# TechnetiumMan/DiffSound

Hardware: AMD Instinct MI355X
Metric: fwd+bwd modal-analysis passes/sec, 100k-tet ord-2 mesh, 64 modes (higher is better)
Workload: dtype f32

## Files before the change

diffsound_amd/csrc/spmm_narrow.inc:

```
constexpr int NARROW_TILE = 320;

template <bool SCALAR, int LVL>
__global__ void __launch_bounds__(256)
    spmm_union_narrow_kernel(const int2* __restrict__ utab, const int4* __restrict__ ctab, unsigned ngroups,
                             const int32_t* __restrict__ gent, const float* __restrict__ vals, int64_t nv,
                             const float* __restrict__ X, int64_t ldx, float* __restrict__ Y, int64_t ldy, int ncols, unsigned nwg) {
    using f4 = __attribute__((ext_vector_type(4))) float;
    __shared__ int s_ent[4][NARROW_TILE];
    __shared__ int s_pre[4][NARROW_TILE];
    const int lane = threadIdx.x & 63;
    const int wave = __builtin_amdgcn_readfirstlane(threadIdx.x >> 6);
    const unsigned grp = ds::xcd_remap(blockIdx.x, nwg) * 4 + wave;
    if (grp >= ngroups) return;
    int ch0 = (int)grp, ch1 = (int)grp + 1;
    if (utab) {
        const int2 ut = utab[grp];
        ch0 = __builtin_amdgcn_readfirstlane(ut.x), ch1 = __builtin_amdgcn_readfirstlane(ut.y);
    }
    const int4 cf = ctab[ch0];
    const int e0 = __builtin_amdgcn_readfirstlane(cf.x);
    const int b0 = __builtin_amdgcn_readfirstlane(cf.z);
    const int e1 = ch1 - 1 == ch0 ? __builtin_amdgcn_readfirstlane(cf.y) : __builtin_amdgcn_readfirstlane(ctab[ch1 - 1].y);
    const int ne = e1 - e0;
    const int cq = ncols >> 2;
    const int sh = cq == 1 ? 0 : (cq == 2 ? 1 : 2);
    const int cl = lane & ((1 << sh) - 1), es = lane >> sh, nslot = 64 >> sh;
    const bool active = cl < cq;
    int* se = s_ent[wave];
    int* sp = s_pre[wave];
    f4 acc[4][3];
#pragma unroll
    for (int s = 0; s < 4; ++s)
#pragma unroll
        for (int i = 0; i < 3; ++i) acc[s][i] = f4{0.f, 0.f, 0.f, 0.f};
    int base_blk = b0;
    for (int t0 = 0; t0 < ne; t0 += NARROW_TILE) {
        const int nt = min(NARROW_TILE, ne - t0);
        int running = 0;
        for (int i = 0; i < nt; i += 64) {
            const int idx = i + lane;
            const int ent = idx < nt ? gent[e0 + t0 + idx] : 0;
            const int pc = __builtin_popcount((unsigned)ent >> 28);
            int incl = pc;
#pragma unroll
            for (int d = 1; d < 64; d <<= 1) {
                const int v = __shfl_up(incl, d);
                if (lane >= d) incl += v;
            }
            if (idx < nt) se[idx] = ent, sp[idx] = running + incl - pc;
            running += __shfl(incl, 63);
        }
        __builtin_amdgcn_fence(__ATOMIC_RELEASE, "wavefront");
        __builtin_amdgcn_wave_barrier();
        __builtin_amdgcn_fence(__ATOMIC_ACQUIRE, "wavefront");
        for (int e = es; e < nt; e += nslot) {
            const int ent = se[e];
            const unsigned m = (unsigned)ent >> 28;
            const int64_t col = ent & 0x0fffffff;
            int64_t blk = base_blk + sp[e];
            f4 x0 = {0.f, 0.f, 0.f, 0.f}, x1 = x0, x2 = x0;
            if (active) {
                const float* xp = X + col * 3 * ldx + cl * 4;
                x0 = *reinterpret_cast<const f4*>(xp);
                x1 = *reinterpret_cast<const f4*>(xp + ldx);
                x2 = *reinterpret_cast<const f4*>(xp + 2 * ldx);
            }
#pragma unroll
            for (int s = 0; s < 4; ++s) {
                if (m & (1u << s)) {
                    if constexpr (SCALAR) {
                        const float c = vals[blk];
                        acc[s][0] += c * x0, acc[s][1] += c * x1, acc[s][2] += c * x2;
                    } else {
                        const float* k = vals + blk * 9;
                        float kk[9];
#pragma unroll
                        for (int j = 0; j < 9; ++j) kk[j] = k[j];
#pragma unroll
                        for (int i = 0; i < 3; ++i) acc[s][i] += kk[i] * x0 + kk[3 + i] * x1 + kk[6 + i] * x2;
                    }
                    ++blk;
                }
            }
        }
        base_blk += running;
        __builtin_amdgcn_fence(__ATOMIC_RELEASE, "wavefront");
        __builtin_amdgcn_wave_barrier();
        __builtin_amdgcn_fence(__ATOMIC_ACQUIRE, "wavefront");
    }
#pragma unroll
    for (int d = 1; d < 64; d <<= 1) {
        if (d >= (1 << sh)) {
#pragma unroll
            for (int s = 0; s < 4; ++s)
#pragma unroll
                for (int i = 0; i < 3; ++i)
#pragma unroll
                    for (int c = 0; c < 4; ++c) acc[s][i][c] += __shfl_xor(acc[s][i][c], d);
        }
    }
    const int64_t n0 = (int64_t)grp * 4;
    const int nn = (int)min<int64_t>(4, nv - n0);
    if (es == 0 && active) {
#pragma unroll
        for (int s = 0; s < 4; ++s)
            if (s < nn) {
#pragma unroll
                for (int i = 0; i < 3; ++i) *reinterpret_cast<f4*>(Y + ((n0 + s) * 3 + i) * ldy + cl * 4) = acc[s][i];
            }
    }
}
```

diffsound_amd/csrc/spmm_union.hip:

```cpp
#include <algorithm>
#include <cstdint>
#include <type_traits>

#include "spmm_device.h"

namespace {
#include "spmm_union.inc"
#include "spmm_narrow.inc"
}

__global__ void pack_groups_kernel(const float* __restrict__ vals_t, const int32_t* __restrict__ kperm, int64_t nnzb,
                                   float* __restrict__ kgrp) {
    const int64_t i = (int64_t)blockIdx.x * blockDim.x + threadIdx.x;
    if (i >= nnzb * 9) return;
    const int64_t p = i / 9;
    kgrp[i] = vals_t[(int64_t)kperm[p] * 9 + (i - p * 9)];
}

extern "C" int ds_pack_groups(const float* vals_t, const int32_t* kperm, int64_t nnzb, float* kgrp,
                              ds_stream_t stream) {
    DS_REQUIRE(vals_t && kperm && kgrp && nnzb > 0, "ds_pack_groups: bad argument");
    pack_groups_kernel<<<(unsigned)ds::ceil_div(nnzb * 9, 256), 256, 0, ds::as_stream(stream)>>>(vals_t, kperm, nnzb,
                                                                                                kgrp);
    DS_LAUNCH_CHECK("pack_groups_kernel");
    return DS_OK;
}

static int check_union_shape(const char* who, int64_t ngroups, int cap_blocks, int64_t nnzb, int64_t nv, int ncols,
                             const char* cap_note = "") {
    DS_REQUIRE(nv > 0 && ngroups == (nv + 3) / 4 && nnzb > 0 && ncols > 0 && ncols % 4 == 0 && ncols <= 84,
               "%s: ncols must be a multiple of 4 <= 84 and ngroups = ceil(nv / 4)", who);
    DS_REQUIRE(cap_blocks > 0 && cap_blocks <= UN_CAPB, "%s: a chunk of %d blocks exceeds the LDS image%s", who, cap_blocks, cap_note);
    return DS_OK;
}

extern "C" int ds_spmm_union(int epilogue, int level_tag, const int32_t* utab, const int32_t* ctab, int64_t ngroups, int cap_blocks,
                             const int32_t* gent,
                             const float* kgrp, int64_t nnzb, int64_t nv, const float* X, int64_t ldx, float* Y,
                             int64_t ldy, const float* R0, int64_t ldr, const float* dinv, int ncols, float c1, float c2,
                             int first, const float* Wprev, int64_t ldp, ds_stream_t stream) {
    DS_REQUIRE(ctab && gent && kgrp && X && Y, "ds_spmm_union: null pointer");
    DS_REQUIRE(epilogue >= 0 && epilogue <= 3, "ds_spmm_union: bad epilogue %d", epilogue);
    DS_REQUIRE(level_tag == 0 || level_tag == 1, "ds_spmm_union: level_tag must be 0 (fine) or 1 (corner-node level)");
    DS_REQUIRE(epilogue == 0 || epilogue == 3 || R0, "ds_spmm_union: the epilogue needs R0");
    DS_REQUIRE(epilogue != 1 || dinv, "ds_spmm_union: the Chebyshev epilogue needs dinv");
    if (int rc = check_union_shape("ds_spmm_union", ngroups, cap_blocks, nnzb, nv, ncols, " (DS_UNION_CAP = 140)")) return rc;
    DS_REQUIRE(ldx >= ncols && ldy >= ncols && (epilogue == 0 || epilogue == 3 || ldr >= ncols),
               "ds_spmm_union: leading dimension smaller than ncols");
    DS_REQUIRE(X != Y, "ds_spmm_union: X and Y must be different buffers");
    DS_REQUIRE(ldx * 12 < (int64_t)PIPE_OOB && ldy * 12 < (int64_t)PIPE_OOB && ldr * 12 < (int64_t)PIPE_OOB &&
                   nv * 36 < (int64_t)PIPE_OOB,
               "ds_spmm_union: a 3-row panel of %lld bytes exceeds the descriptor range", (long long)(ldx * 12));
    DS_REQUIRE(nnzb * 36 < ((int64_t)1 << 32), "ds_spmm_union: value array exceeds the descriptor range");
    uintptr_t al = reinterpret_cast<uintptr_t>(X) | reinterpret_cast<uintptr_t>(Y) | (uintptr_t)(ldx * 4) |
                   (uintptr_t)(ldy * 4) | reinterpret_cast<uintptr_t>(kgrp) | reinterpret_cast<uintptr_t>(ctab);
    if (epilogue == 1 || epilogue == 2) al |= reinterpret_cast<uintptr_t>(R0) | (uintptr_t)(ldr * 4);
    DS_REQUIRE((al & 15) == 0, "ds_spmm_union: rows, kgrp and ctab must be 16-byte aligned");
    hipStream_t st = ds::as_stream(stream);
    ChebEpilogue epi{R0, ldr, dinv, c1, c2, first};
    if (Wprev && epilogue == 1) {
        DS_REQUIRE(ldp >= ncols && ldp * 12 < (int64_t)PIPE_OOB &&
                       ((reinterpret_cast<uintptr_t>(Wprev) | (uintptr_t)(ldp * 4)) & 15) == 0 && Wprev != X,
                   "ds_spmm_union: bad W_prev block");
        epi.wprev = Wprev, epi.ldp = ldp;
    }
    const int lpn = ncols / 4;
    const int pkind = epilogue == 1 ? DS_PROF_TERM : (epilogue == 0 ? DS_PROF_KX : (epilogue == 3 ? DS_PROF_MX : -1));
    ds::ProfScope prof(pkind < 0 ? nullptr : stream, pkind < 0 ? 0 : pkind, nv, nnzb, ncols, (first ? 1 : 0) | (4 << 8));
#define DS_U(L, E) return launch_union<L, E>(utab, ctab, ngroups, cap_blocks, gent, kgrp, nnzb, nv, X, ldx, Y, ldy, lpn, st, epi)
#define DS_UL(L, E) do { if (level_tag == 1) return launch_union<L, E, false, true, 1>(utab, ctab, ngroups, cap_blocks, gent, kgrp, nnzb, nv, X, ldx, Y, ldy, lpn, st, epi); \
                         return launch_union<L, E, false, true, 0>(utab, ctab, ngroups, cap_blocks, gent, kgrp, nnzb, nv, X, ldx, Y, ldy, lpn, st, epi); } while (0)
    if (lpn == 20) {
        if (epilogue == 1) DS_U(20, 1);
        if (epilogue == 2) DS_U(20, 2);
        if (epilogue == 3) DS_UL(20, 3);
        DS_UL(20, 0);
    }
    if (epilogue == 1) DS_U(0, 1);
    if (epilogue == 2) DS_U(0, 2);
    if (epilogue == 3) DS_UL(0, 3);
    DS_UL(0, 0);
#undef DS_UL
#undef DS_U
}

extern "C" int ds_spmm_union_narrow(int kind, int level_tag, const int32_t* utab, const int32_t* ctab, int64_t ngroups,
                                    const int32_t* gent, const float* vals, int64_t nnzb, int64_t nv, const float* X, int64_t ldx,
                                    float* Y, int64_t ldy, int ncols, ds_stream_t stream) {
    DS_REQUIRE(ctab && gent && vals && X && Y, "ds_spmm_union_narrow: null pointer");
    DS_REQUIRE(kind == 0 || kind == 3, "ds_spmm_union_narrow: kind must be 0 (3x3 blocks) or 3 (node-scalar values)");
    DS_REQUIRE(level_tag == 0 || level_tag == 1, "ds_spmm_union_narrow: level_tag must be 0 (fine) or 1 (corner-node level)");
    DS_REQUIRE(nv > 0 && ngroups == (nv + 3) / 4 && nnzb > 0 && ncols > 0 && ncols % 4 == 0 && ncols <= 16,
               "ds_spmm_union_narrow: ncols must be a multiple of 4 <= 16 and ngroups = ceil(nv / 4)");
    DS_REQUIRE(ldx >= ncols && ldy >= ncols, "ds_spmm_union_narrow: leading dimension smaller than ncols");
    DS_REQUIRE(X != Y, "ds_spmm_union_narrow: X and Y must be different buffers");
    const uintptr_t al = reinterpret_cast<uintptr_t>(X) | reinterpret_cast<uintptr_t>(Y) | (uintptr_t)(ldx * 4) | (uintptr_t)(ldy * 4) |
                         reinterpret_cast<uintptr_t>(ctab);
    DS_REQUIRE((al & 15) == 0, "ds_spmm_union_narrow: rows and ctab must be 16-byte aligned");
    hipStream_t st = ds::as_stream(stream);
    const unsigned nwg = (unsigned)ds::ceil_div(ngroups, 4);
    ds::ProfScope prof(stream, kind == 0 ? DS_PROF_KX : DS_PROF_MX, nv, nnzb, ncols, 4 << 8);
#define DS_UN(S, V) spmm_union_narrow_kernel<S, V><<<nwg, 256, 0, st>>>(reinterpret_cast<const int2*>(utab), reinterpret_cast<const int4*>(ctab), \
                                                                       (unsigned)ngroups, gent, vals, nv, X, ldx, Y, ldy, ncols, nwg)
    if (kind == 0) {
        if (level_tag == 1) DS_UN(false, 1);
        else DS_UN(false, 0);
    } else {
        if (level_tag == 1) DS_UN(true, 1);
        else DS_UN(true, 0);
    }
#undef DS_UN
    DS_LAUNCH_CHECK("spmm_union_narrow_kernel");
    return DS_OK;
}

extern "C" int64_t ds_union_residual_workspace_bytes(int64_t ngroups, int ncols) {
    return ngroups * 2 * (int64_t)ncols * 4 + (int64_t)UN_NORM_BLOCKS * 2 * ncols * 8;
}

static int union_residual(const char* who, int level_tag, const int32_t* utab, const int32_t* ctab, int64_t ngroups, int cap_blocks,
                          const int32_t* gent, const float* kgrp, const float* mgrp, int64_t nnzb, int64_t nv, const float* X,
                          int64_t ldx, const double* lam, float* R, int64_t ldr, const float* dinv, float c, void* R16,
                          int64_t ldr16, void* W1, int64_t ldw1, int ncols, void* work, int64_t work_bytes, double* rn2,
                          double* xn2, ds_stream_t stream) {
    const bool pre = R16 != nullptr;
    DS_REQUIRE(ctab && gent && kgrp && mgrp && X && lam && (pre ? (W1 && dinv) : R != nullptr) && work && rn2 && xn2, "%s: null pointer", who);
    DS_REQUIRE(level_tag == 0 || (level_tag == 1 && !pre), "%s: level_tag must be 0 (fine)%s", who, pre ? "" : " or 1 (corner-node level)");
    if (int rc = check_union_shape(who, ngroups, cap_blocks, nnzb, nv, ncols)) return rc;
    uintptr_t al = reinterpret_cast<uintptr_t>(X) | (uintptr_t)(ldx * 4) | reinterpret_cast<uintptr_t>(kgrp) |
                   reinterpret_cast<uintptr_t>(ctab) | reinterpret_cast<uintptr_t>(work);
    if (pre) {
        DS_REQUIRE(ldx >= ncols && ldr16 >= ncols && ldw1 >= ncols, "%s: leading dimension smaller than ncols", who);
        DS_REQUIRE(R16 != W1 && R16 != X && W1 != X, "%s: X, R16 and W1 must be different buffers", who);
        DS_REQUIRE(ldx * 12 < (int64_t)PIPE_OOB && nv * 36 < (int64_t)PIPE_OOB && nnzb * 36 < ((int64_t)1 << 32),
                   "%s: operand beyond the descriptor range", who);
        const uintptr_t al8 = reinterpret_cast<uintptr_t>(R16) | reinterpret_cast<uintptr_t>(W1) | (uintptr_t)(ldr16 * 2) | (uintptr_t)(ldw1 * 2);
        DS_REQUIRE((al8 & 7) == 0 && (reinterpret_cast<uintptr_t>(dinv) & 3) == 0, "%s: bf16 rows must be 8-byte aligned", who);
    } else {
        DS_REQUIRE(ldx >= ncols && ldr >= ncols, "%s: leading dimension smaller than ncols", who);
        DS_REQUIRE(X != R, "%s: X and R must be different buffers", who);
        DS_REQUIRE(ldx * 12 < (int64_t)PIPE_OOB && ldr * 12 < (int64_t)PIPE_OOB && nnzb * 36 < ((int64_t)1 << 32),
                   "%s: operand beyond the descriptor range", who);
        al |= reinterpret_cast<uintptr_t>(R) | (uintptr_t)(ldr * 4);
    }
    DS_REQUIRE((al & 15) == 0, "%s: rows, kgrp, ctab and the workspace must be 16-byte aligned", who);
    DS_REQUIRE(work_bytes >= ds_union_residual_workspace_bytes(ngroups, ncols), "%s: workspace of %lld bytes needed", who,
               (long long)ds_union_residual_workspace_bytes(ngroups, ncols));
    hipStream_t st = ds::as_stream(stream);
    ChebEpilogue epi{nullptr, 0, pre ? dinv : nullptr, 0.f, pre ? c : 0.f, 0};
    epi.mvals = mgrp, epi.lam = lam, epi.nwork = static_cast<float*>(work);
    epi.w1 = W1, epi.ldw1 = ldw1;
    float* Y = pre ? static_cast<float*>(R16) : R;
    const int64_t ldy = pre ? ldr16 : ldr;
    const int lpn = ncols / 4;
    int rc;
    {
    ds::ProfScope prof(stream, DS_PROF_RESID, nv, nnzb, ncols, 4 << 8);
#define DS_UR(L, E, V) rc = launch_union<L, E, false, true, V>(utab, ctab, ngroups, cap_blocks, gent, kgrp, nnzb, nv, X, ldx, Y, ldy, lpn, st, epi)
    if (lpn == 20) {
        if (pre) DS_UR(20, 6, 0);
        else if (level_tag == 1) DS_UR(20, 4, 1);
        else DS_UR(20, 4, 0);
    } else {
        if (pre) DS_UR(0, 6, 0);
        else if (level_tag == 1) DS_UR(0, 4, 1);
        else DS_UR(0, 4, 0);
    }
#undef DS_UR
    }
    if (rc != DS_OK) return rc;
    double* partial = reinterpret_cast<double*>(static_cast<char*>(work) + ngroups * 2 * (int64_t)ncols * 4);
    union_norm_partial_kernel<<<UN_NORM_BLOCKS, 256, 0, st>>>(static_cast<const float*>(work), (unsigned)ngroups, 2 * ncols, partial);
    DS_LAUNCH_CHECK("union_norm_partial_kernel");
    union_norm_final_kernel<<<(unsigned)(2 * ncols), 256, 0, st>>>(partial, ncols, rn2, xn2);
    DS_LAUNCH_CHECK("union_norm_final_kernel");
    return DS_OK;
}

extern "C" int ds_union_residual(int level_tag, const int32_t* utab, const int32_t* ctab, int64_t ngroups, int cap_blocks,
                                 const int32_t* gent, const float* kgrp, const float* mgrp, int64_t nnzb, int64_t nv,
                                 const float* X, int64_t ldx, const double* lam, float* R, int64_t ldr, int ncols, void* work,
                                 int64_t work_bytes, double* rn2, double* xn2, ds_stream_t stream) {
    return union_residual("ds_union_residual", level_tag, utab, ctab, ngroups, cap_blocks, gent, kgrp, mgrp, nnzb, nv, X, ldx, lam, R,
                          ldr, nullptr, 0.f, nullptr, 0, nullptr, 0, ncols, work, work_bytes, rn2, xn2, stream);
}

extern "C" int ds_union_residual_pre(int level_tag, const int32_t* utab, const int32_t* ctab, int64_t ngroups, int cap_blocks,
                                     const int32_t* gent, const float* kgrp, const float* mgrp, int64_t nnzb, int64_t nv,
                                     const float* X, int64_t ldx, const double* lam, const float* dinv, float c, void* R16,
                                     int64_t ldr16, void* W1, int64_t ldw1, int ncols, void* work, int64_t work_bytes,
                                     double* rn2, double* xn2, ds_stream_t stream) {
    DS_REQUIRE(R16, "ds_union_residual_pre: null pointer");
    return union_residual("ds_union_residual_pre", level_tag, utab, ctab, ngroups, cap_blocks, gent, kgrp, mgrp, nnzb, nv, X, ldx, lam,
                          nullptr, 0, dinv, c, R16, ldr16, W1, ldw1, ncols, work, work_bytes, rn2, xn2, stream);
}

extern "C" int ds_spmm_union_km(int level_tag, const int32_t* utab, const int32_t* ctab, int64_t ngroups, int cap_blocks,
                                const int32_t* gent, const float* kgrp, const float* mgrp, int64_t nnzb, int64_t nv,
                                const float* X, int64_t ldx, float* KX, int64_t ldk, float* MX, int64_t ldm, int ncols,
                                ds_stream_t stream) {
    DS_REQUIRE(ctab && gent && kgrp && mgrp && X && KX && MX, "ds_spmm_union_km: null pointer");
    DS_REQUIRE(level_tag == 0 || level_tag == 1, "ds_spmm_union_km: level_tag must be 0 (fine) or 1 (corner-node level)");
    if (int rc = check_union_shape("ds_spmm_union_km", ngroups, cap_blocks, nnzb, nv, ncols)) return rc;
    DS_REQUIRE(ldx >= ncols && ldk >= ncols && ldm >= ncols, "ds_spmm_union_km: leading dimension smaller than ncols");
    DS_REQUIRE(X != KX && X != MX && KX != MX, "ds_spmm_union_km: X, KX and MX must be different buffers");
    DS_REQUIRE(ldx * 12 < (int64_t)PIPE_OOB && nnzb * 36 < ((int64_t)1 << 32), "ds_spmm_union_km: operand beyond the descriptor range");
    const uintptr_t al = reinterpret_cast<uintptr_t>(X) | reinterpret_cast<uintptr_t>(KX) | reinterpret_cast<uintptr_t>(MX) |
                         (uintptr_t)(ldx * 4) | (uintptr_t)(ldk * 4) | (uintptr_t)(ldm * 4) | reinterpret_cast<uintptr_t>(kgrp) |
                         reinterpret_cast<uintptr_t>(ctab);
    DS_REQUIRE((al & 15) == 0, "ds_spmm_union_km: rows, kgrp and ctab must be 16-byte aligned");
    hipStream_t st = ds::as_stream(stream);
    ChebEpilogue epi{nullptr, ldm, nullptr, 0.f, 0.f, 0};
    epi.mvals = mgrp, epi.nwork = MX;
    const int lpn = ncols / 4;
    ds::ProfScope prof(stream, DS_PROF_KM, nv, nnzb, ncols, 4 << 8);
#define DS_UKM(L, V) return launch_union<L, 5, false, true, V>(utab, ctab, ngroups, cap_blocks, gent, kgrp, nnzb, nv, X, ldx, KX, ldk, lpn, st, epi)
    if (lpn == 20) {
        if (level_tag == 1) DS_UKM(20, 1);
        DS_UKM(20, 0);
    }
    if (level_tag == 1) DS_UKM(0, 1);
    DS_UKM(0, 0);
#undef DS_UKM
}

extern "C" int ds_spmm_union16(int epilogue, const int32_t* utab, const int32_t* ctab, int64_t ngroups, int cap_blocks,
                               const int32_t* gent, const float* kgrp, int64_t nnzb, int64_t nv, const void* X,
                               int64_t ldx, void* Y, int64_t ldy, int y_f32, const void* R0, int64_t ldr,
                               const float* dinv, int ncols, float c1, float c2, int first, const void* Wprev,
                               int64_t ldp, ds_stream_t stream) {
    DS_REQUIRE(ctab && gent && kgrp && X && Y && R0, "ds_spmm_union16: null pointer");
    DS_REQUIRE(epilogue == 1 || epilogue == 2, "ds_spmm_union16: epilogue must be 1 (Chebyshev term) or 2 (residual)");
    DS_REQUIRE(epilogue != 1 || dinv, "ds_spmm_union16: the Chebyshev epilogue needs dinv");
    if (int rc = check_union_shape("ds_spmm_union16", ngroups, cap_blocks, nnzb, nv, ncols)) return rc;
    DS_REQUIRE(ldx >= ncols && ldy >= ncols && ldr >= ncols, "ds_spmm_union16: leading dimension smaller than ncols");
    DS_REQUIRE(X != Y, "ds_spmm_union16: X and Y must be different buffers");
    DS_REQUIRE(3 * nv * std::max(std::max(ldx, ldr), ldp) * 2 < (int64_t)PIPE_OOB && nv * 36 < (int64_t)PIPE_OOB,
               "ds_spmm_union16: a bf16 operand block of %lld bytes exceeds the descriptor range",
               (long long)(3 * nv * std::max(std::max(ldx, ldr), ldp) * 2));
    DS_REQUIRE(nnzb * 36 < ((int64_t)1 << 32), "ds_spmm_union16: value array exceeds the descriptor range");
    uintptr_t al = reinterpret_cast<uintptr_t>(X) | reinterpret_cast<uintptr_t>(R0) | (uintptr_t)(ldx * 2) | (uintptr_t)(ldr * 2);
    al |= reinterpret_cast<uintptr_t>(Y) | (uintptr_t)(ldy * (y_f32 ? 4 : 2));
    DS_REQUIRE((al & 7) == 0 && (!y_f32 || ((reinterpret_cast<uintptr_t>(Y) | (uintptr_t)(ldy * 4)) & 15) == 0) &&
                   ((reinterpret_cast<uintptr_t>(kgrp) | reinterpret_cast<uintptr_t>(ctab)) & 15) == 0,
               "ds_spmm_union16: bf16 rows must be 8-byte aligned (fp32 output rows, kgrp and ctab 16-byte)");
    hipStream_t st = ds::as_stream(stream);
    ChebEpilogue epi{static_cast<const float*>(R0), ldr, dinv, c1, c2, first};
    if (Wprev && epilogue == 1) {
        DS_REQUIRE(ldp >= ncols && ((reinterpret_cast<uintptr_t>(Wprev) | (uintptr_t)(ldp * 2)) & 7) == 0 && Wprev != X,
                   "ds_spmm_union16: bad W_prev block");
        epi.wprev = static_cast<const float*>(Wprev), epi.ldp = ldp;
    }
    DS_REQUIRE(!y_f32 || epilogue == 1, "ds_spmm_union16: an fp32 result is the Chebyshev term's only");
    const float* Xf = static_cast<const float*>(X);
    float* Yf = static_cast<float*>(Y);
    const int lpn = ncols / 4;
    ds::ProfScope prof((epilogue == 1 && !y_f32) ? stream : nullptr, DS_PROF_TERM, nv, nnzb, ncols, (first ? 1 : 0) | (2 << 8));
#define DS_U16(L, E, O) return launch_union<L, E, true, O>(utab, ctab, ngroups, cap_blocks, gent, kgrp, nnzb, nv, Xf, ldx, Yf, ldy, lpn, st, epi)
    if (lpn == 20) {
        if (epilogue == 2) DS_U16(20, 2, false);
        if (y_f32) DS_U16(20, 1, true);
        DS_U16(20, 1, false);
    }
    if (epilogue == 2) DS_U16(0, 2, false);
    if (y_f32) DS_U16(0, 1, true);
    DS_U16(0, 1, false);
#undef DS_U16
}
```

Baseline: 70.68.

## Stage narrow SpMM block values in LDS with coalesced loads and prefetch X

The narrow union SpMM kernel now loads each tile's matrix values with coalesced 16-byte loads into per-wave shared memory and bounds each tile by both an entry count and a block budget. It also software-pipelines the X row loads one entry ahead, replaces the full butterfly reduction with a slot-splitting transpose reduction so fewer shuffles are needed before the store, and adds an occupancy hint to launch bounds. This targets the scattered per-lane global reads of 3x3 blocks and the shuffle cost of the final reduction. In exchange it uses more LDS per block, takes smaller tiles (more loop iterations and barriers), and adds misalignment handling.

```diff
diff --git a/diffsound_amd/csrc/spmm_narrow.inc b/diffsound_amd/csrc/spmm_narrow.inc
--- a/diffsound_amd/csrc/spmm_narrow.inc
+++ b/diffsound_amd/csrc/spmm_narrow.inc
@@ -1,13 +1,59 @@
-constexpr int NARROW_TILE = 320;
+constexpr int NARROW_TILE = 128;
+constexpr int NARROW_VB = 160;
+constexpr int NARROW_VIMG = NARROW_VB * 9 + 8;
+
+using narrow_f4 = __attribute__((ext_vector_type(4))) float;
+
+template <int SH>
+__device__ __forceinline__ void narrow_slot_sum_store(narrow_f4 (&acc)[4][3], int lane, int cl, bool active, int nn, float* __restrict__ Y,
+                                                      int64_t n0, int64_t ldy) {
+    using f4 = narrow_f4;
+    constexpr int DA = 1 << SH, DB = 2 << SH;
+    const bool hia = (lane & DA) != 0, hib = (lane & DB) != 0;
+    f4 r[2][3];
+#pragma unroll
+    for (int s = 0; s < 2; ++s)
+#pragma unroll
+        for (int i = 0; i < 3; ++i) {
+            f4 keep = hia ? acc[2 + s][i] : acc[s][i];
+            const f4 send = hia ? acc[s][i] : acc[2 + s][i];
+#pragma unroll
+            for (int c = 0; c < 4; ++c) keep[c] += __shfl_xor(send[c], DA);
+            r[s][i] = keep;
+        }
+    f4 q[3];
+#pragma unroll
+    for (int i = 0; i < 3; ++i) {
+        f4 keep = hib ? r[1][i] : r[0][i];
+        const f4 send = hib ? r[0][i] : r[1][i];
+#pragma unroll
+        for (int c = 0; c < 4; ++c) keep[c] += __shfl_xor(send[c], DB);
+        q[i] = keep;
+    }
+#pragma unroll
+    for (int d = 4 << SH; d < 64; d <<= 1)
+#pragma unroll
+        for (int i = 0; i < 3; ++i)
+#pragma unroll
+            for (int c = 0; c < 4; ++c) q[i][c] += __shfl_xor(q[i][c], d);
+    const int s = (hia ? 2 : 0) + (hib ? 1 : 0);
+    if (lane < (4 << SH) && active && s < nn) {
+#pragma unroll
+        for (int i = 0; i < 3; ++i) *reinterpret_cast<f4*>(Y + ((n0 + s) * 3 + i) * ldy + cl * 4) = q[i];
+    }
+}
 
 template <bool SCALAR, int LVL>
-__global__ void __launch_bounds__(256)
+__global__ void __launch_bounds__(256, 4)
     spmm_union_narrow_kernel(const int2* __restrict__ utab, const int4* __restrict__ ctab, unsigned ngroups,
-                             const int32_t* __restrict__ gent, const float* __restrict__ vals, int64_t nv,
+                             const int32_t* __restrict__ gent, const float* __restrict__ vals, int64_t nvals, int64_t nv,
                              const float* __restrict__ X, int64_t ldx, float* __restrict__ Y, int64_t ldy, int ncols, unsigned nwg) {
-    using f4 = __attribute__((ext_vector_type(4))) float;
+    using f4 = narrow_f4;
+    constexpr int EPB = SCALAR ? 1 : 9;
+    constexpr int VROUNDS = (NARROW_VIMG / 4 + 63) / 64;
     __shared__ int s_ent[4][NARROW_TILE];
     __shared__ int s_pre[4][NARROW_TILE];
+    __shared__ __attribute__((aligned(16))) float s_val[4][NARROW_VIMG];
     const int lane = threadIdx.x & 63;
     const int wave = __builtin_amdgcn_readfirstlane(threadIdx.x >> 6);
     const unsigned grp = ds::xcd_remap(blockIdx.x, nwg) * 4 + wave;
@@ -20,7 +66,11 @@
     const int4 cf = ctab[ch0];
     const int e0 = __builtin_amdgcn_readfirstlane(cf.x);
     const int b0 = __builtin_amdgcn_readfirstlane(cf.z);
-    const int e1 = ch1 - 1 == ch0 ? __builtin_amdgcn_readfirstlane(cf.y) : __builtin_amdgcn_readfirstlane(ctab[ch1 - 1].y);
+    int e1 = __builtin_amdgcn_readfirstlane(cf.y), bend = __builtin_amdgcn_readfirstlane(cf.w);
+    if (ch1 - 1 != ch0) {
+        const int4 cl4 = ctab[ch1 - 1];
+        e1 = __builtin_amdgcn_readfirstlane(cl4.y), bend = __builtin_amdgcn_readfirstlane(cl4.w);
+    }
     const int ne = e1 - e0;
     const int cq = ncols >> 2;
     const int sh = cq == 1 ? 0 : (cq == 2 ? 1 : 2);
@@ -28,85 +78,121 @@
     const bool active = cl < cq;
     int* se = s_ent[wave];
     int* sp = s_pre[wave];
+    float* sv = s_val[wave];
     f4 acc[4][3];
 #pragma unroll
     for (int s = 0; s < 4; ++s)
 #pragma unroll
         for (int i = 0; i < 3; ++i) acc[s][i] = f4{0.f, 0.f, 0.f, 0.f};
     int base_blk = b0;
-    for (int t0 = 0; t0 < ne; t0 += NARROW_TILE) {
-        const int nt = min(NARROW_TILE, ne - t0);
-        int running = 0;
-        for (int i = 0; i < nt; i += 64) {
-            const int idx = i + lane;
-            const int ent = idx < nt ? gent[e0 + t0 + idx] : 0;
-            const int pc = __builtin_popcount((unsigned)ent >> 28);
-            int incl = pc;
+    for (int t0 = 0; t0 < ne;) {
+        int entr[NARROW_TILE / 64];
 #pragma unroll
-            for (int d = 1; d < 64; d <<= 1) {
-                const int v = __shfl_up(incl, d);
-                if (lane >= d) incl += v;
+        for (int r = 0; r < NARROW_TILE / 64; ++r) {
+            const int g = t0 + r * 64 + lane;
+            entr[r] = g < ne ? gent[e0 + g] : 0;
+        }
+        const int nbst = min(NARROW_VB, bend - base_blk);
+        const int64_t f0 = (int64_t)base_blk * EPB;
+        const int mis = __builtin_amdgcn_readfirstlane((int)((reinterpret_cast<uintptr_t>(vals + f0) >> 2) & 3));
+        const int nq = (mis + nbst * EPB + 3) >> 2;
+        f4 vst[VROUNDS];
+#pragma unroll
+        for (int r = 0; r < VROUNDS; ++r) {
+            const int qi = r * 64 + lane;
+            vst[r] = f4{0.f, 0.f, 0.f, 0.f};
+            if (qi < nq) {
+                const int64_t gi = f0 - mis + 4 * (int64_t)qi;
+                if (gi >= 0 && gi + 4 <= nvals) {
+                    vst[r] = *reinterpret_cast<const f4*>(vals + gi);
+                } else {
+#pragma unroll
+                    for (int c = 0; c < 4; ++c)
+                        if (gi + c >= 0 && gi + c < nvals) vst[r][c] = vals[gi + c];
+                }
             }
-            if (idx < nt) se[idx] = ent, sp[idx] = running + incl - pc;
-            running += __shfl(incl, 63);
+        }
+        int nt = 0, running = 0;
+#pragma unroll
+        for (int r = 0; r < NARROW_TILE / 64; ++r) {
+            if (nt == r * 64 && t0 + r * 64 < ne) {
+                const int idx = r * 64 + lane;
+                const int ent = entr[r];
+                const int pc = __builtin_popcount((unsigned)ent >> 28);
+                int incl = pc;
+#pragma unroll
+                for (int d = 1; d < 64; d <<= 1) {
+                    const int v = __shfl_up(incl, d);
+                    if (lane >= d) incl += v;
+                }
+                const bool ok = t0 + idx < ne && running + incl <= nbst;
+                if (ok) se[idx] = ent, sp[idx] = running + incl - pc;
+                const int nfit = __builtin_popcountll(__ballot(ok));
+                if (nfit) running += __shfl(incl, nfit - 1);
+                nt += nfit;
+            }
+        }
+        if (nt == 0) break;
+#pragma unroll
+        for (int r = 0; r < VROUNDS; ++r) {
+            const int qi = r * 64 + lane;
+            if (qi < nq) *reinterpret_cast<f4*>(sv + 4 * qi) = vst[r];
         }
         __builtin_amdgcn_fence(__ATOMIC_RELEASE, "wavefront");
         __builtin_amdgcn_wave_barrier();
         __builtin_amdgcn_fence(__ATOMIC_ACQUIRE, "wavefront");
-        for (int e = es; e < nt; e += nslot) {
-            const int ent = se[e];
+        int e = es;
+        int ent = e < nt ? se[e] : 0;
+        int pre = e < nt ? sp[e] : 0;
+        f4 x0 = {0.f, 0.f, 0.f, 0.f}, x1 = x0, x2 = x0;
+        if (e < nt && active) {
+            const float* xp = X + (int64_t)(ent & 0x0fffffff) * 3 * ldx + cl * 4;
+            x0 = *reinterpret_cast<const f4*>(xp);
+            x1 = *reinterpret_cast<const f4*>(xp + ldx);
+            x2 = *reinterpret_cast<const f4*>(xp + 2 * ldx);
+        }
+        while (e < nt) {
+            const int en = e + nslot;
+            const bool more = en < nt;
+            const int entn = more ? se[en] : 0;
+            const int pren = more ? sp[en] : 0;
+            f4 y0 = {0.f, 0.f, 0.f, 0.f}, y1 = y0, y2 = y0;
+            if (more && active) {
+                const float* xp = X + (int64_t)(entn & 0x0fffffff) * 3 * ldx + cl * 4;
+                y0 = *reinterpret_cast<const f4*>(xp);
+                y1 = *reinterpret_cast<const f4*>(xp + ldx);
+                y2 = *reinterpret_cast<const f4*>(xp + 2 * ldx);
+            }
             const unsigned m = (unsigned)ent >> 28;
-            const int64_t col = ent & 0x0fffffff;
-            int64_t blk = base_blk + sp[e];
-            f4 x0 = {0.f, 0.f, 0.f, 0.f}, x1 = x0, x2 = x0;
-            if (active) {
-                const float* xp = X + col * 3 * ldx + cl * 4;
-                x0 = *reinterpret_cast<const f4*>(xp);
-                x1 = *reinterpret_cast<const f4*>(xp + ldx);
-                x2 = *reinterpret_cast<const f4*>(xp + 2 * ldx);
-            }
+            const float* k = sv + mis + pre * EPB;
 #pragma unroll
             for (int s = 0; s < 4; ++s) {
                 if (m & (1u << s)) {
                     if constexpr (SCALAR) {
-                        const float c = vals[blk];
+                        const float c = k[0];
                         acc[s][0] += c * x0, acc[s][1] += c * x1, acc[s][2] += c * x2;
                     } else {
-                        const float* k = vals + blk * 9;
-                        float kk[9];
 #pragma unroll
-                        for (int j = 0; j < 9; ++j) kk[j] = k[j];
+                        for (int i = 0; i < 3; ++i) acc[s][i] += k[i] * x0;
 #pragma unroll
-                        for (int i = 0; i < 3; ++i) acc[s][i] += kk[i] * x0 + kk[3 + i] * x1 + kk[6 + i] * x2;
+                        for (int i = 0; i < 3; ++i) acc[s][i] += k[3 + i] * x1;
+#pragma unroll
+                        for (int i = 0; i < 3; ++i) acc[s][i] += k[6 + i] * x2;
                     }
-                    ++blk;
+                    k += EPB;
                 }
             }
+            ent = entn, pre = pren, x0 = y0, x1 = y1, x2 = y2, e = en;
         }
+        t0 += nt;
         base_blk += running;
         __builtin_amdgcn_fence(__ATOMIC_RELEASE, "wavefront");
         __builtin_amdgcn_wave_barrier();
         __builtin_amdgcn_fence(__ATOMIC_ACQUIRE, "wavefront");
     }
-#pragma unroll
-    for (int d = 1; d < 64; d <<= 1) {
-        if (d >= (1 << sh)) {
-#pragma unroll
-            for (int s = 0; s < 4; ++s)
-#pragma unroll
-                for (int i = 0; i < 3; ++i)
-#pragma unroll
-                    for (int c = 0; c < 4; ++c) acc[s][i][c] += __shfl_xor(acc[s][i][c], d);
-        }
-    }
     const int64_t n0 = (int64_t)grp * 4;
     const int nn = (int)min<int64_t>(4, nv - n0);
-    if (es == 0 && active) {
-#pragma unroll
-        for (int s = 0; s < 4; ++s)
-            if (s < nn) {
-#pragma unroll
-                for (int i = 0; i < 3; ++i) *reinterpret_cast<f4*>(Y + ((n0 + s) * 3 + i) * ldy + cl * 4) = acc[s][i];
-            }
-    }
+    if (sh == 0) narrow_slot_sum_store<0>(acc, lane, cl, active, nn, Y, n0, ldy);
+    else if (sh == 1) narrow_slot_sum_store<1>(acc, lane, cl, active, nn, Y, n0, ldy);
+    else narrow_slot_sum_store<2>(acc, lane, cl, active, nn, Y, n0, ldy);
 }
diff --git a/diffsound_amd/csrc/spmm_union.hip b/diffsound_amd/csrc/spmm_union.hip
--- a/diffsound_amd/csrc/spmm_union.hip
+++ b/diffsound_amd/csrc/spmm_union.hip
@@ -101,7 +101,7 @@
     const unsigned nwg = (unsigned)ds::ceil_div(ngroups, 4);
     ds::ProfScope prof(stream, kind == 0 ? DS_PROF_KX : DS_PROF_MX, nv, nnzb, ncols, 4 << 8);
 #define DS_UN(S, V) spmm_union_narrow_kernel<S, V><<<nwg, 256, 0, st>>>(reinterpret_cast<const int2*>(utab), reinterpret_cast<const int4*>(ctab), \
-                                                                       (unsigned)ngroups, gent, vals, nv, X, ldx, Y, ldy, ncols, nwg)
+                                                                       (unsigned)ngroups, gent, vals, nnzb * (S ? 1 : 9), nv, X, ldx, Y, ldy, ncols, nwg)
     if (kind == 0) {
         if (level_tag == 1) DS_UN(false, 1);
         else DS_UN(false, 0);
```

Result: no change. 70.30 (-0.5%).
